# ViV99/slam-experiments

Hardware: AMD Instinct MI355X
Metric: descriptor pairs/sec BF-Hamming knn=2 @64kx64k (higher is better)
Workload: dtype u32

## Files before the change

slam-experiments_amd/csrc/bf_mx.hip:

```cpp
#include "internal.h"
#include <vector>
#include <atomic>
#include <type_traits>

#include "bf_common.h"

#define SLAM_MX_STAGE 128
#define SLAM_MX_BOUND_LIMIT 0x7F000000u
#define SLAM_MX_EARLY 0x16u
#define SLAM_MX_UNROLL 4
#define SLAM_MX_RESIDENT 4

typedef int mx_v8i __attribute__((ext_vector_type(8)));
typedef float mx_v4f __attribute__((ext_vector_type(4)));

__device__ __forceinline__ uint4 mx_expand(u32 x) {
    uint4 r;
    r.x = ((x << 3) & 0x88888888u) | 0x22222222u;
    r.y = ((x << 2) & 0x88888888u) | 0x22222222u;
    r.z = ((x << 1) & 0x88888888u) | 0x22222222u;
    r.w = (x & 0x88888888u) | 0x22222222u;
    return r;
}

__device__ __forceinline__ mx_v4f mx_dot(uint4 a, uint4 b, mx_v4f c) {
    const mx_v8i av = {(int)a.x, (int)a.y, (int)a.z, (int)a.w, 0, 0, 0, 0};
    const mx_v8i bv = {(int)b.x, (int)b.y, (int)b.z, (int)b.w, 0, 0, 0, 0};
    return __builtin_amdgcn_mfma_scale_f32_16x16x128_f8f6f4(av, bv, c, 4, 4, 0, 127, 0, 127);
}

__device__ __forceinline__ void mx_unite(u32& b1, u32& b2, u32 c1, u32 c2) {
    const u32 n2 = min(max(b1, c1), min(b2, c2));
    b1 = min(b1, c1);
    b2 = n2;
}

__device__ __forceinline__ u32 mx_pick(const u32 (&v)[4], int i) {
    return i == 0 ? v[0] : (i == 1 ? v[1] : (i == 2 ? v[2] : v[3]));
}

__global__ __launch_bounds__(256) void bf_top2_mx_kernel(const uint4* __restrict__ q, int N, const uint4* __restrict__ t,
                                                         const int* __restrict__ tbl, bf_state st, int train_base,
                                                         int2* __restrict__ out_idx, int2* __restrict__ out_dist,
                                                         uint4* __restrict__ keep, int nchunks, bf_select sel) {
    __shared__ uint4 tile[2][SLAM_MX_STAGE * 8];
    __shared__ u32 s_ticket, s_last;
    const int tid = threadIdx.x;
    const int lane = tid & 63, wave = tid >> 6;
    const int kg = lane >> 4, col = lane & 15;
    const u32 lanek = (u32)(4 * kg - (1 << SLAM_KEY_IDX_BITS));
    const int bx = ((int)blockIdx.x + (int)blockIdx.y) % (int)gridDim.x;
    const int qbase = bx * 256 + wave * 64 + lane;

    uint4 qb[4][2];
    const u32* qw = (const u32*)q;
#pragma unroll
    for (int tt = 0; tt < 4; tt++) {
        int qi = bx * 256 + wave * 64 + tt * 16 + col;
        qi = qi < N ? qi : N - 1;
#pragma unroll
        for (int h = 0; h < 2; h++) qb[tt][h] = mx_expand(qw[(size_t)qi * 8 + h * 4 + kg]);
    }
    if (keep && blockIdx.y == 0 && qbase < N) {
        keep[2 * (size_t)qbase] = q[2 * (size_t)qbase];
        keep[2 * (size_t)qbase + 1] = q[2 * (size_t)qbase + 1];
    }

    u32 b1[4], b2[4], x[4];
    mx_v4f cth[4];
    auto set_threshold = [&](int tt) {
        const float c = (float)(2 * (int)x[tt] - 258);
        cth[tt] = mx_v4f{c, c, c, c};
    };
#pragma unroll
    for (int tt = 0; tt < 4; tt++) {
        b1[tt] = b2[tt] = SLAM_KEY_NONE;
        x[tt] = SLAM_KEY_NONE >> SLAM_KEY_IDX_BITS;
        set_threshold(tt);
    }
    auto unite_tile = [&](int tt, u32& u1, u32& u2) {
        u1 = b1[tt];
        u2 = b2[tt];
#pragma unroll
        for (int off = 16; off <= 32; off <<= 1) {
            const u32 c1 = (u32)__shfl_xor((int)u1, off, 64), c2 = (u32)__shfl_xor((int)u2, off, 64);
            mx_unite(u1, u2, c1, c2);
        }
    };
    auto unite_lanes = [&](u32 (&u1)[4], u32 (&u2)[4]) {
#pragma unroll
        for (int tt = 0; tt < 4; tt++) unite_tile(tt, u1[tt], u2[tt]);
    };
    u32 gkey = SLAM_BOUND_IDLE, pend[1] = {0u};
    auto exchange = [&](int c0) {
        u32 u1[4], u2[4];
        unite_lanes(u1, u2);
        if (qbase < N) {
            const u32 own = mx_pick(u2, kg);
            asm volatile("" ::"v"(pend[0]));
            const u32 g = __hip_atomic_load(&st.bound[qbase], __ATOMIC_RELAXED, __HIP_MEMORY_SCOPE_AGENT);
            if (own < g && own < SLAM_MX_BOUND_LIMIT) pend[0] = atomicMin(&st.bound[qbase], own);
            gkey = g;
        }
#pragma unroll
        for (int tt = 0; tt < 4; tt++) {
            const u32 g = (u32)__shfl((int)gkey, tt * 16 + col, 64);
            const u32 gx = g < SLAM_MX_BOUND_LIMIT ? (g >> SLAM_KEY_IDX_BITS) + ((g & SLAM_KEY_IDX_MASK) < (u32)c0 ? 0u : 1u)
                                                   : SLAM_KEY_NONE >> SLAM_KEY_IDX_BITS;
            x[tt] = min(x[tt], min(gx, u2[tt] >> SLAM_KEY_IDX_BITS));
            set_threshold(tt);
        }
    };

    const int srow = tid >> 1, sh = tid & 1;
    auto load_stage = [&](int s, int c1) -> uint4 {
        const uint4* ts = t + 2 * (size_t)s;
        if (s + SLAM_MX_STAGE <= c1) return ts[(u32)tid];
        return s + srow < c1 ? ts[(u32)tid] : make_uint4(0, 0, 0, 0);
    };
    const u32 fill = 0x22222222u;
    auto expand = [&](u32 v) -> uint4 {
        uint4 r;
        asm("v_and_or_b32 %0, %1, %2, %3" : "=v"(r.x) : "v"(v << 3), "s"(0x88888888u), "v"(fill));
        asm("v_and_or_b32 %0, %1, %2, %3" : "=v"(r.y) : "v"(v << 2), "s"(0x88888888u), "v"(fill));
        asm("v_and_or_b32 %0, %1, %2, %3" : "=v"(r.z) : "v"(v << 1), "s"(0x88888888u), "v"(fill));
        asm("v_and_or_b32 %0, %1, %2, %3" : "=v"(r.w) : "v"(v), "s"(0x88888888u), "v"(fill));
        return r;
    };
    uint4* const dst0 = tile[0] + (srow >> 4) * 128 + sh * 64 + (srow & 15);
    auto store_stage = [&](int b, uint4 v) {
        uint4* dst = dst0 + b * (SLAM_MX_STAGE * 8);
        dst[0] = expand(v.x);
        dst[16] = expand(v.y);
        dst[32] = expand(v.z);
        dst[48] = expand(v.w);
    };

    u32* const cursor = st.cursor + (size_t)(4 * bx) * SLAM_CURSOR_STRIDE;
    if (tid == 0) s_ticket = __hip_atomic_fetch_add(cursor, 1u, __ATOMIC_RELAXED, __HIP_MEMORY_SCOPE_AGENT);
    __syncthreads();
    int ci = __builtin_amdgcn_readfirstlane((int)s_ticket);
    int scanned = 0;
    while (ci < nchunks) {
        const int c0 = tbl[ci], c1 = tbl[ci + 1];
        uint4 nx = load_stage(c0, c1);
        exchange(c0);
        store_stage(0, nx);
        __syncthreads();
        int buf = 0;
        for (int s0 = c0; s0 < c1; s0 += SLAM_MX_STAGE) {
            const int s1 = s0 + SLAM_MX_STAGE;
            const bool more = s1 < c1;
            if (more) nx = load_stage(s1, c1);
            else if (tid == 0) s_ticket = __hip_atomic_fetch_add(cursor, 1u, __ATOMIC_RELAXED, __HIP_MEMORY_SCOPE_AGENT);
            const int ng = __builtin_amdgcn_readfirstlane(min(SLAM_MX_STAGE / 16, (c1 - s0 + 15) >> 4));
            const uint4* tp = tile[buf];
            u32 fired = 0;
            auto group = [&](int g, auto rag) {
                const uint4 a0 = tp[g * 128 + lane], a1 = tp[g * 128 + 64 + lane];
                mx_v4f acc[4];
#pragma unroll
                for (int tt = 0; tt < 4; tt++) acc[tt] = mx_dot(a0, qb[tt][0], cth[tt]);
#pragma unroll
                for (int tt = 0; tt < 4; tt++) acc[tt] = mx_dot(a1, qb[tt][1], acc[tt]);
                int p[4];
#pragma unroll
                for (int tt = 0; tt < 4; tt++)
                    p[tt] = max(max(__float_as_int(acc[tt][0]), __float_as_int(acc[tt][1])), __float_as_int(acc[tt][2]));
                int m = max(max(p[0], __float_as_int(acc[0][3])), p[1]);
                m = max(max(m, __float_as_int(acc[1][3])), p[2]);
                m = max(max(m, __float_as_int(acc[2][3])), p[3]);
                m = max(m, __float_as_int(acc[3][3]));
                if (__builtin_expect(__ballot(m >= 0) != 0ull, 0)) {
                    const u32 rowk = (u32)__builtin_amdgcn_readfirstlane(s0 + g * 16) + lanek;
#pragma unroll
                    for (int tt = 0; tt < 4; tt++) {
                        if (__ballot(max(p[tt], __float_as_int(acc[tt][3])) >= 0) == 0ull) continue;
                        fired |= 1u << tt;
                        const u32 base = (x[tt] << SLAM_KEY_IDX_BITS) + rowk;
#pragma unroll
                        for (int r = 0; r < 4; r++) {
                            if (__ballot(__float_as_int(acc[tt][r]) >= 0) == 0ull) continue;
                            u32 key = base + (u32)r + ((u32)(int)(-acc[tt][r]) << (SLAM_KEY_IDX_BITS - 1));
                            if constexpr (decltype(rag)::value)
                                key = (int)rowk + r < c1 - (1 << SLAM_KEY_IDX_BITS) ? key : SLAM_KEY_NONE;
                            b2[tt] = umed3(b1[tt], b2[tt], key);
                            b1[tt] = min(b1[tt], key);
                        }
                        x[tt] = min(x[tt], b2[tt] >> SLAM_KEY_IDX_BITS);
                        set_threshold(tt);
                    }
                }
            };
            const int nwhole = __builtin_amdgcn_readfirstlane(min(SLAM_MX_STAGE / 16, (c1 - s0) >> 4));
            int g = 0;
            for (; g + SLAM_MX_UNROLL <= nwhole; g += SLAM_MX_UNROLL) {
#pragma unroll
                for (int k = 0; k < SLAM_MX_UNROLL; k++) {
                    group(g + k, std::false_type{});
                    __builtin_amdgcn_sched_barrier(0);
                }
            }
            for (; g < ng; g++) group(g, std::true_type{});
#pragma unroll
            for (int tt = 0; tt < 4; tt++) {
                if (!(fired >> tt & 1u)) continue;
                u32 u1, u2;
                unite_tile(tt, u1, u2);
                x[tt] = min(x[tt], u2 >> SLAM_KEY_IDX_BITS);
                set_threshold(tt);
            }
            scanned += min(s1, c1) - s0;
            if (more && scanned < 32 * SLAM_MX_STAGE && (SLAM_MX_EARLY >> (scanned / SLAM_MX_STAGE) & 1u)) exchange(s1);
            if (more) store_stage(buf ^ 1, nx);
            __syncthreads();
            buf ^= 1;
        }
        ci = __builtin_amdgcn_readfirstlane((int)s_ticket);
    }

    u32 u1[4], u2[4];
    unite_lanes(u1, u2);
    const u32 f1[1] = {mx_pick(u1, kg)}, f2[1] = {mx_pick(u2, kg)};
    const u32 gk[1] = {gkey < SLAM_MX_BOUND_LIMIT ? gkey >> SLAM_KEY_IDX_BITS : SLAM_BOUND_IDLE};
    bf_top2_epilogue<1, true>(st, bx, tid, lane, qbase, false, false, f1, f2, gk, pend, N, (int)gridDim.y, train_base, out_idx,
                              out_dist, sel, s_last);
}


struct bf_mx_plan {
    int qblocks;
    int workers;
    int chunk;
    int S;
    int tail;
};

static bf_mx_plan make_mx_plan_core(int num_cu, int resident, int64_t N, int64_t M, std::vector<int>* tbl) {
    bf_mx_plan p;
    p.qblocks = (int)((N + 255) / 256);
    int64_t W = (int64_t)num_cu * resident / p.qblocks;
    if (W < 1) W = 1;
    if (W > 256) W = 256;
    const int64_t c = M / W >= 8192 ? 1024 : 256;
    std::vector<int>& b = *tbl;
    b.clear();
    b.push_back(0);
    int shrinking = 0;
    for (int64_t at = 0; at < M;) {
        int64_t len = c;
        const int64_t g = (M - at) / (2 * W) / SLAM_MX_STAGE * SLAM_MX_STAGE;
        if (g < len) { len = g < SLAM_MX_STAGE ? SLAM_MX_STAGE : g; shrinking++; }
        at = at + len < M ? at + len : M;
        b.push_back((int)at);
    }
    p.chunk = (int)c;
    p.S = (int)b.size() - 1;
    p.tail = shrinking;
    p.workers = (int)(W < p.S ? W : p.S);
    return p;
}

static bool bf_mx_auto(int64_t N, int64_t M) {
    return (N >= 8192 && M >= 16384) || (N >= 3000 && M >= 40000) || (N >= 1000 && M >= 65536) || (N >= 500 && M >= 200000);
}

extern "C" int slam_bf_mx_plan_describe(int num_cu, int64_t N, int64_t M, int32_t* h_plan, int32_t* h_tbl, int64_t tbl_cap,
                                        int64_t* tbl_len) {
    SLAM_REQUIRE(num_cu >= 1 && num_cu <= 4096, "num_cu out of range");
    SLAM_REQUIRE(N >= 1 && M >= 1 && M <= SLAM_MAX_TRAIN_PER_PASS && N <= (1ll << 30), "bad sizes");
    SLAM_REQUIRE(h_plan && tbl_len && (h_tbl || tbl_cap == 0) && tbl_cap >= 0, "slam_bf_mx_plan_describe: null argument");
    std::vector<int> tbl;
    const bf_mx_plan p = make_mx_plan_core(num_cu, SLAM_MX_RESIDENT, N, M, &tbl);
    h_plan[0] = p.qblocks; h_plan[1] = p.workers; h_plan[2] = p.chunk; h_plan[3] = p.S;
    h_plan[4] = p.tail; h_plan[5] = SLAM_MX_STAGE; h_plan[6] = SLAM_MX_RESIDENT; h_plan[7] = bf_mx_auto(N, M) ? 1 : 0;
    *tbl_len = (int64_t)tbl.size();
    for (int64_t i = 0; i < (int64_t)tbl.size() && i < tbl_cap; i++) h_tbl[i] = tbl[(size_t)i];
    return SLAM_OK;
}

extern "C" int slam_bf_set_engine(slam_ctx* ctx, int engine) {
    SLAM_REQUIRE(ctx, "slam_bf_set_engine: null ctx");
    SLAM_REQUIRE(engine >= 0 && engine <= 2, "engine must be 0 (auto), 1 (VALU) or 2 (matrix cores where eligible)");
    std::lock_guard<std::mutex> g(ctx->mu);
    ctx->bf_engine = engine;
    return SLAM_OK;
}

bool bf_mx_route(slam_ctx* ctx, int64_t N, int64_t M, bool rows_on_host) {
    std::lock_guard<std::mutex> g(ctx->mu);
    if (ctx->bf_engine == 1 || rows_on_host) return false;
    for (int i = 0; i < SLAM_BF_KNOBS; i++)
        if (ctx->bf_knob[i]) return false;
    return ctx->bf_engine == 2 || bf_mx_auto(N, M);
}

int bf_mx_pass(slam_ctx* ctx, const void* d_query, int64_t N, const void* d_train, int64_t M, int64_t train_base, int32_t* d_idx,
               int32_t* d_dist, void* d_keep, const bf_select& sel, int* qblocks_out) {
    static std::atomic<int> occ_once{0};
    int occ = occ_once.load(std::memory_order_relaxed);
    if (!occ) {
        int o = 0;
        SLAM_HIP(hipOccupancyMaxActiveBlocksPerMultiprocessor(&o, bf_top2_mx_kernel, 256, 0));
        occ = o > 0 ? o : SLAM_MX_RESIDENT;
        occ_once.store(occ, std::memory_order_relaxed);
    }
    std::vector<int> tbl;
    int num_cu;
    {
        std::lock_guard<std::mutex> g(ctx->mu);
        num_cu = ctx->num_cu;
    }
    const bf_mx_plan p = make_mx_plan_core(num_cu, occ, N, M, &tbl);
    bf_state st;
    if (int rc = bf_state_get(ctx, N, &st)) return rc;
    const int* d_tbl = nullptr;
    if (int rc = bf_table_get(ctx, tbl, &d_tbl)) return rc;
    if (qblocks_out) *qblocks_out = p.qblocks;
    SLAM_HIP(hipGetLastError());
    if (int rc = slam_prof_begin(ctx)) return rc;
    bf_top2_mx_kernel<<<dim3(p.qblocks, p.workers), dim3(256), 0, ctx->stream>>>(
        (const uint4*)d_query, (int)N, (const uint4*)d_train, d_tbl, st, (int)train_base, (int2*)d_idx, (int2*)d_dist,
        (uint4*)d_keep, p.S, sel);
    if (int rc = slam_prof_end(ctx)) return rc;
    const hipError_t e = hipGetLastError();
    if (e != hipSuccess) {
        (void)bf_state_reset(ctx);
        return slam_set_error(SLAM_ERR_HIP, "top-2 MX kernel launch failed: %s", hipGetErrorString(e));
    }
    return SLAM_OK;
}
```

Before: 10340 billion.

## Interleave next-stage train loads and expansion into MFMA loop, trim VGPR state

The kernel no longer loads the whole next stage into a register up front and stores it after compute. Instead the next stage's words are loaded during the last groups of the current stage, and the bit expansion plus LDS store are interleaved between MFMA calls under sched_barriers. It also frees VGPRs: the per-tile x is now recovered from the threshold float, qbase is recomputed on demand, and waves_per_eu is pinned to 4. This is meant to hide global-load and expansion latency behind matrix math and keep occupancy, at the cost of some extra ALU work and a more rigid schedule.

```diff
diff --git a/slam-experiments_amd/csrc/bf_mx.hip b/slam-experiments_amd/csrc/bf_mx.hip
--- a/slam-experiments_amd/csrc/bf_mx.hip
+++ b/slam-experiments_amd/csrc/bf_mx.hip
@@ -39,7 +39,7 @@
     return i == 0 ? v[0] : (i == 1 ? v[1] : (i == 2 ? v[2] : v[3]));
 }
 
-__global__ __launch_bounds__(256) void bf_top2_mx_kernel(const uint4* __restrict__ q, int N, const uint4* __restrict__ t,
+__global__ __launch_bounds__(256) __attribute__((amdgpu_waves_per_eu(4, 4))) void bf_top2_mx_kernel(const uint4* __restrict__ q, int N, const uint4* __restrict__ t,
                                                          const int* __restrict__ tbl, bf_state st, int train_base,
                                                          int2* __restrict__ out_idx, int2* __restrict__ out_dist,
                                                          uint4* __restrict__ keep, int nchunks, bf_select sel) {
@@ -50,7 +50,11 @@
     const int kg = lane >> 4, col = lane & 15;
     const u32 lanek = (u32)(4 * kg - (1 << SLAM_KEY_IDX_BITS));
     const int bx = ((int)blockIdx.x + (int)blockIdx.y) % (int)gridDim.x;
-    const int qbase = bx * 256 + wave * 64 + lane;
+    auto lane_query = [&]() -> int {
+        int v = tid;
+        asm volatile("" : "+v"(v));
+        return bx * 256 + v;
+    };
 
     uint4 qb[4][2];
     const u32* qw = (const u32*)q;
@@ -61,22 +65,22 @@
 #pragma unroll
         for (int h = 0; h < 2; h++) qb[tt][h] = mx_expand(qw[(size_t)qi * 8 + h * 4 + kg]);
     }
-    if (keep && blockIdx.y == 0 && qbase < N) {
+    if (const int qbase = lane_query(); keep && blockIdx.y == 0 && qbase < N) {
         keep[2 * (size_t)qbase] = q[2 * (size_t)qbase];
         keep[2 * (size_t)qbase + 1] = q[2 * (size_t)qbase + 1];
     }
 
-    u32 b1[4], b2[4], x[4];
+    u32 b1[4], b2[4];
     mx_v4f cth[4];
-    auto set_threshold = [&](int tt) {
-        const float c = (float)(2 * (int)x[tt] - 258);
+    auto set_threshold = [&](int tt, u32 x) {
+        const float c = (float)(2 * (int)x - 258);
         cth[tt] = mx_v4f{c, c, c, c};
     };
+    auto threshold_x = [&](int tt) -> u32 { return (u32)((int)cth[tt][0] + 258) >> 1; };
 #pragma unroll
     for (int tt = 0; tt < 4; tt++) {
         b1[tt] = b2[tt] = SLAM_KEY_NONE;
-        x[tt] = SLAM_KEY_NONE >> SLAM_KEY_IDX_BITS;
-        set_threshold(tt);
+        set_threshold(tt, SLAM_KEY_NONE >> SLAM_KEY_IDX_BITS);
     }
     auto unite_tile = [&](int tt, u32& u1, u32& u2) {
         u1 = b1[tt];
@@ -95,7 +99,7 @@
     auto exchange = [&](int c0) {
         u32 u1[4], u2[4];
         unite_lanes(u1, u2);
-        if (qbase < N) {
+        if (const int qbase = lane_query(); qbase < N) {
             const u32 own = mx_pick(u2, kg);
             asm volatile("" ::"v"(pend[0]));
             const u32 g = __hip_atomic_load(&st.bound[qbase], __ATOMIC_RELAXED, __HIP_MEMORY_SCOPE_AGENT);
@@ -107,8 +111,7 @@
             const u32 g = (u32)__shfl((int)gkey, tt * 16 + col, 64);
             const u32 gx = g < SLAM_MX_BOUND_LIMIT ? (g >> SLAM_KEY_IDX_BITS) + ((g & SLAM_KEY_IDX_MASK) < (u32)c0 ? 0u : 1u)
                                                    : SLAM_KEY_NONE >> SLAM_KEY_IDX_BITS;
-            x[tt] = min(x[tt], min(gx, u2[tt] >> SLAM_KEY_IDX_BITS));
-            set_threshold(tt);
+            set_threshold(tt, min(threshold_x(tt), min(gx, u2[tt] >> SLAM_KEY_IDX_BITS)));
         }
     };
 
@@ -143,26 +146,23 @@
     int scanned = 0;
     while (ci < nchunks) {
         const int c0 = tbl[ci], c1 = tbl[ci + 1];
-        uint4 nx = load_stage(c0, c1);
+        const uint4 first = load_stage(c0, c1);
         exchange(c0);
-        store_stage(0, nx);
+        store_stage(0, first);
         __syncthreads();
         int buf = 0;
         for (int s0 = c0; s0 < c1; s0 += SLAM_MX_STAGE) {
             const int s1 = s0 + SLAM_MX_STAGE;
             const bool more = s1 < c1;
-            if (more) nx = load_stage(s1, c1);
-            else if (tid == 0) s_ticket = __hip_atomic_fetch_add(cursor, 1u, __ATOMIC_RELAXED, __HIP_MEMORY_SCOPE_AGENT);
+            if (!more && tid == 0) s_ticket = __hip_atomic_fetch_add(cursor, 1u, __ATOMIC_RELAXED, __HIP_MEMORY_SCOPE_AGENT);
             const int ng = __builtin_amdgcn_readfirstlane(min(SLAM_MX_STAGE / 16, (c1 - s0 + 15) >> 4));
             const uint4* tp = tile[buf];
             u32 fired = 0;
-            auto group = [&](int g, auto rag) {
-                const uint4 a0 = tp[g * 128 + lane], a1 = tp[g * 128 + 64 + lane];
-                mx_v4f acc[4];
-#pragma unroll
-                for (int tt = 0; tt < 4; tt++) acc[tt] = mx_dot(a0, qb[tt][0], cth[tt]);
-#pragma unroll
-                for (int tt = 0; tt < 4; tt++) acc[tt] = mx_dot(a1, qb[tt][1], acc[tt]);
+            auto dots0 = [&](const uint4& a, mx_v4f (&acc)[4]) {
+#pragma unroll
+                for (int tt = 0; tt < 4; tt++) acc[tt] = mx_dot(a, qb[tt][0], cth[tt]);
+            };
+            auto fold = [&](int g, mx_v4f (&acc)[4], auto rag) {
                 int p[4];
 #pragma unroll
                 for (int tt = 0; tt < 4; tt++)
@@ -172,12 +172,15 @@
                 m = max(max(m, __float_as_int(acc[2][3])), p[3]);
                 m = max(m, __float_as_int(acc[3][3]));
                 if (__builtin_expect(__ballot(m >= 0) != 0ull, 0)) {
-                    const u32 rowk = (u32)__builtin_amdgcn_readfirstlane(s0 + g * 16) + lanek;
+                    int row0 = s0 + g * 16;
+                    asm("" : "+s"(row0));
+                    const u32 rowk = (u32)row0 + lanek;
 #pragma unroll
                     for (int tt = 0; tt < 4; tt++) {
                         if (__ballot(max(p[tt], __float_as_int(acc[tt][3])) >= 0) == 0ull) continue;
                         fired |= 1u << tt;
-                        const u32 base = (x[tt] << SLAM_KEY_IDX_BITS) + rowk;
+                        const u32 xt = threshold_x(tt);
+                        const u32 base = (xt << SLAM_KEY_IDX_BITS) + rowk;
 #pragma unroll
                         for (int r = 0; r < 4; r++) {
                             if (__ballot(__float_as_int(acc[tt][r]) >= 0) == 0ull) continue;
@@ -187,32 +190,85 @@
                             b2[tt] = umed3(b1[tt], b2[tt], key);
                             b1[tt] = min(b1[tt], key);
                         }
-                        x[tt] = min(x[tt], b2[tt] >> SLAM_KEY_IDX_BITS);
-                        set_threshold(tt);
+                        set_threshold(tt, min(xt, b2[tt] >> SLAM_KEY_IDX_BITS));
                     }
+                }
+            };
+            auto group = [&](int g, auto rag) {
+                const uint4 a0 = tp[g * 128 + lane], a1 = tp[g * 128 + 64 + lane];
+                mx_v4f acc[4];
+                dots0(a0, acc);
+#pragma unroll
+                for (int tt = 0; tt < 4; tt++) acc[tt] = mx_dot(a1, qb[tt][1], acc[tt]);
+                fold(g, acc, rag);
+            };
+            auto trip = [&](int g0, auto ngc, auto shadow) {
+                constexpr int NG = decltype(ngc)::value;
+                constexpr bool SH = decltype(shadow)::value;
+                const uint4* ap = tp + g0 * 128 + lane;
+                uint4* const dst = dst0 + (buf ^ 1) * (SLAM_MX_STAGE * 8);
+                const u32* nw = (const u32*)(t + 2 * (size_t)s1) + 8 * min(srow, c1 - 1 - s1) + 4 * sh;
+                u32 w = 0;
+                uint4 a0 = ap[0], a1 = ap[64];
+#pragma unroll
+                for (int k = 0; k < NG; k++) {
+                    uint4 a0n = a0, a1n = a1;
+                    mx_v4f acc[4];
+                    if (k + 1 < NG) a0n = ap[(k + 1) * 128];
+                    const u32 v = w;
+                    if (SH && k >= NG - 5 && k < NG - 1) w = nw[k - (NG - 5)];
+                    __builtin_amdgcn_sched_barrier(0);
+                    dots0(a0, acc);
+                    __builtin_amdgcn_sched_barrier(0);
+                    if (SH && k >= NG - 4) {
+                        const int j = k - (NG - 4);
+                        uint4 e;
+                        acc[0] = mx_dot(a1, qb[0][1], acc[0]);
+                        __builtin_amdgcn_sched_barrier(0);
+                        asm volatile("v_lshlrev_b32 %0, 3, %1\n\tv_and_or_b32 %0, %0, %2, %3" : "=v"(e.x) : "v"(v), "s"(0x88888888u), "v"(fill));
+                        asm volatile("v_lshlrev_b32 %0, 2, %1" : "=v"(e.y) : "v"(v));
+                        __builtin_amdgcn_sched_barrier(0);
+                        acc[1] = mx_dot(a1, qb[1][1], acc[1]);
+                        __builtin_amdgcn_sched_barrier(0);
+                        asm volatile("v_and_or_b32 %0, %1, %2, %3" : "=v"(e.y) : "v"(e.y), "s"(0x88888888u), "v"(fill));
+                        asm volatile("v_lshlrev_b32 %0, 1, %1\n\tv_and_or_b32 %0, %0, %2, %3" : "=v"(e.z) : "v"(v), "s"(0x88888888u), "v"(fill));
+                        __builtin_amdgcn_sched_barrier(0);
+                        acc[2] = mx_dot(a1, qb[2][1], acc[2]);
+                        __builtin_amdgcn_sched_barrier(0);
+                        asm volatile("v_and_or_b32 %0, %1, %2, %3" : "=v"(e.w) : "v"(v), "s"(0x88888888u), "v"(fill));
+                        dst[16 * j] = e;
+                        if (k + 1 < NG) a1n = ap[(k + 1) * 128 + 64];
+                        __builtin_amdgcn_sched_barrier(0);
+                        acc[3] = mx_dot(a1, qb[3][1], acc[3]);
+                    } else {
+                        if (k + 1 < NG) a1n = ap[(k + 1) * 128 + 64];
+                        __builtin_amdgcn_sched_barrier(0);
+#pragma unroll
+                        for (int tt = 0; tt < 4; tt++) acc[tt] = mx_dot(a1, qb[tt][1], acc[tt]);
+                    }
+                    fold(g0 + k, acc, std::false_type{});
+                    __builtin_amdgcn_sched_barrier(0);
+                    a0 = a0n;
+                    a1 = a1n;
                 }
             };
             const int nwhole = __builtin_amdgcn_readfirstlane(min(SLAM_MX_STAGE / 16, (c1 - s0) >> 4));
             int g = 0;
-            for (; g + SLAM_MX_UNROLL <= nwhole; g += SLAM_MX_UNROLL) {
-#pragma unroll
-                for (int k = 0; k < SLAM_MX_UNROLL; k++) {
-                    group(g + k, std::false_type{});
-                    __builtin_amdgcn_sched_barrier(0);
-                }
+            if (more) {
+                trip(0, std::integral_constant<int, SLAM_MX_STAGE / 16>{}, std::true_type{});
+                g = SLAM_MX_STAGE / 16;
             }
+            for (; g + SLAM_MX_UNROLL <= nwhole; g += SLAM_MX_UNROLL) trip(g, std::integral_constant<int, SLAM_MX_UNROLL>{}, std::false_type{});
             for (; g < ng; g++) group(g, std::true_type{});
 #pragma unroll
             for (int tt = 0; tt < 4; tt++) {
                 if (!(fired >> tt & 1u)) continue;
                 u32 u1, u2;
                 unite_tile(tt, u1, u2);
-                x[tt] = min(x[tt], u2 >> SLAM_KEY_IDX_BITS);
-                set_threshold(tt);
+                set_threshold(tt, min(threshold_x(tt), u2 >> SLAM_KEY_IDX_BITS));
             }
             scanned += min(s1, c1) - s0;
             if (more && scanned < 32 * SLAM_MX_STAGE && (SLAM_MX_EARLY >> (scanned / SLAM_MX_STAGE) & 1u)) exchange(s1);
-            if (more) store_stage(buf ^ 1, nx);
             __syncthreads();
             buf ^= 1;
         }
@@ -223,7 +279,7 @@
     unite_lanes(u1, u2);
     const u32 f1[1] = {mx_pick(u1, kg)}, f2[1] = {mx_pick(u2, kg)};
     const u32 gk[1] = {gkey < SLAM_MX_BOUND_LIMIT ? gkey >> SLAM_KEY_IDX_BITS : SLAM_BOUND_IDLE};
-    bf_top2_epilogue<1, true>(st, bx, tid, lane, qbase, false, false, f1, f2, gk, pend, N, (int)gridDim.y, train_base, out_idx,
+    bf_top2_epilogue<1, true>(st, bx, tid, lane, lane_query(), false, false, f1, f2, gk, pend, N, (int)gridDim.y, train_base, out_idx,
                               out_dist, sel, s_last);
 }
 
```

Result: faster. 10610 billion (median of 6 runs) (+2.6%).
